# Juzhan/TAP-Net

Hardware: AMD Instinct MI355X
Metric: env-steps/s (batch placements) 2D n=10 LB_GREEDY; 1/2/4/8 GPU + CPU ref (higher is better)
Workload: dtype i32 height-maps / f64 candidate scores / f32 masks

## Files before the change

tap-net_amd/csrc/tap_masks.h:

```cpp
#pragma once

#include <hip/hip_runtime.h>

#include <cstdint>
#include <type_traits>
#include <cstdlib>

#include "tap_stream_variant.h"

constexpr size_t TAP_WT_MAX_BYTES = 64u << 20;

struct MaskArgs {
    int B, n, R, nR, rows, update_rows, static_rows;
    const float *dyn_in;
    float *dyn_out;
    const float *static_;
    const int64_t *ptr;
    const float *mask_in;
    const float *cs_in;
    float *cs_out;
    float *cur_out;
    float *mask_out;
    const unsigned long long *bits_in;
    unsigned long long *bits_out;
// ... 176 lines not shown
{
    const int nR = a.nR;
    const size_t slab = (size_t)a.rows * nR;
    const int nchunk = (int)(slab / 4);
    int total = 0;
#pragma unroll
    for (int k = 0; k < NS; ++k) if (on[k]) total = (k + 1) * nchunk;
    if (total == 0) return;
    long p[NS];
    float row0[NS][NC], cs[NS][NC][3], keep[NS][NC];
#pragma unroll
    for (int k = 0; k < NS; ++k) {
        const int env = senv0 + k;
        p[k] = on[k] ? (long)a.ptr[env] : 0;
#pragma unroll
        for (int c = 0; c < NC; ++c) {
            const int j = lane + 64 * c;
            const bool ok = on[k] && j < nR;
            row0[k][c] = ok ? a.static_[(size_t)env * a.static_rows * nR + j] : 0.f;
            keep[k][c] = ok ? (a.mask_in ? a.mask_in[(size_t)env * nR + j] : 1.f) : 0.f;
#pragma unroll
            for (int s = 0; s < 3; ++s) cs[k][c][s] = ok ? a.cs_in[((size_t)env * 3 + s) * nR + j] : 0.f;
        }
    }
    for (int i = lane; i < NS * 3 * nR; i += 64) lds[i] = 0.f;

    const float4 *s4 = reinterpret_cast<const float4 *>(a.dyn_in + (size_t)senv0 * slab);
    float4 *d4 = reinterpret_cast<float4 *>(a.dyn_out + (size_t)senv0 * slab);
    ClearRanges cr[NS];
    bool have_real = false;
    for (int base = 0; base < total; base += 64 * U) {
        float4 v[U];
#pragma unroll
        for (int u = 0; u < U; ++u) v[u] = s4[min(base + u * 64 + lane, total - 1)];
        if (!have_real) {
#pragma unroll
            for (int k = 0; k < NS; ++k) {
                float r0 = -1.f;
#pragma unroll
                for (int c = 0; c < NC; ++c) {
                    const float t = __shfl(row0[k][c], (int)(p[k] & 63));
                    if ((p[k] >> 6) == c && p[k] >= 0 && p[k] < nR) r0 = t;
                }
                cr[k] = clear_ranges(a, on[k] ? (long)r0 : -1);
            }
            have_real = true;
        }
#pragma unroll
        for (int u = 0; u < U; ++u) {
            const int q = base + u * 64 + lane;
            if (q < total) {
                const int k = (NS > 1 && q >= nchunk) ? 1 : 0;
                const int f = (q - k * nchunk) * 4;
#pragma unroll
                for (int s = 0; s < 3; ++s)
                    if (f >= cr[k].lo[s] && f < cr[k].hi[s]) {
                        *reinterpret_cast<float4 *>(lds + (k * 3 + s) * nR + (f - cr[k].lo[s])) = v[u];
                        v[u] = make_float4(0.f, 0.f, 0.f, 0.f);
                    }
                d4[q] = v[u];
            }
        }
    }
    __builtin_amdgcn_fence(__ATOMIC_RELEASE, "wavefront");
    __builtin_amdgcn_wave_barrier();
    __builtin_amdgcn_fence(__ATOMIC_ACQUIRE, "wavefront");
#pragma unroll
    for (int k = 0; k < NS; ++k) {
        if (!on[k]) continue;
        const int env = senv0 + k;
        const long real_m = (p[k] >= 0 && p[k] < nR) ? tap_mod_col(p[k], a.n, a.nR) : -1 - (long)a.n * a.R;
#pragma unroll
        for (int c = 0; c < NC; ++c) {
            const int j = lane + 64 * c;
            if (j >= nR) continue;
            float sum[3];
#pragma unroll
            for (int s = 0; s < 3; ++s) {
                sum[s] = cs[k][c][s] - lds[(k * 3 + s) * nR + j];
                if (a.cs_out) a.cs_out[((size_t)env * 3 + s) * nR + j] = sum[s];
            }
            float kp = keep[k][c];
            for (int r = 0; r < a.R; ++r)
                if (j == real_m + (long)a.n * r) kp = 0.f;
            if (a.mask_out) a.mask_out[(size_t)env * nR + j] = kp;
            const float dm = sum[1] * sum[2] + sum[0];
            if (a.cur_out) a.cur_out[(size_t)env * nR + j] = dm != 0.f ? 0.f : kp;
        }
    }
}

template <int NS>
__device__ __forceinline__ void stream_build_bits(const MaskArgs &a, int senv0, int lane, const bool (&on)[NS],
                                                  unsigned long long *tile )
{
    typedef unsigned long long u64;
    const int nR = a.nR, C4 = nR >> 2, rows = a.rows;
    const int rsub = (int)(((unsigned)lane * (unsigned)a.c4_magic) >> 16), c4 = lane - rsub * C4, RP = a.rp;
    for (int i = lane; i < NS * nR; i += 64) tile[i] = 0ull;
    tap_wave_lds_sync_m();
    int bad = 0;
    constexpr int U = 4;
    for (int r0 = rsub; r0 < rows; r0 += U * RP) {
        float4 v[NS][U];
#pragma unroll
        for (int k = 0; k < NS; ++k) {
            const float4 *src = reinterpret_cast<const float4 *>(a.dyn_in + (size_t)(senv0 + (on[k] ? k : 0)) * rows * nR) + c4;
#pragma unroll
            for (int u = 0; u < U; ++u) v[k][u] = src[(size_t)min(r0 + u * RP, rows - 1) * C4];
        }
#pragma unroll
        for (int k = 0; k < NS; ++k) {
            unsigned lo[4] = {0u, 0u, 0u, 0u}, hi[4] = {0u, 0u, 0u, 0u};
#pragma unroll
            for (int u = 0; u < U; ++u) {
                const int r = r0 + u * RP;
                if (r >= rows || rsub >= RP || !on[k]) continue;
                const float e[4] = {v[k][u].x, v[k][u].y, v[k][u].z, v[k][u].w};
#pragma unroll
                for (int q = 0; q < 4; ++q) {
                    const unsigned nz = e[q] != 0.f;
                    bad += (nz && e[q] != 1.f);
                    if (r < 32) lo[q] |= nz << r; else hi[q] |= nz << (r - 32);
                }
            }
            if (on[k] && rsub < RP) {
#pragma unroll
                for (int q = 0; q < 4; ++q) {
                    const u64 word = ((u64)hi[q] << 32) | lo[q];
                    if (word) atomicOr(&tile[k * nR + c4 * 4 + q], word);
                }
            }
        }
    }
    if (a.nonbinary) {
        const unsigned long long any = __ballot(bad != 0);
        if (any) {
#pragma unroll
            for (int o = 32; o > 0; o >>= 1) bad += __shfl_xor(bad, o);
            if (lane == 0) atomicAdd(a.nonbinary, bad);
        }
    }
    tap_wave_lds_sync_m();
}

__device__ __forceinline__ int tap_mod_small(int v, int n)
{
#pragma unroll
    for (int r = 0; r < 5; ++r) v = v >= n ? v - n : v;
    while (v >= n) v -= n;
    return v;
}

template <int NS, int NC, bool BUILD = false, bool MERGED = true, int C4S = 0, bool INPLACE = false, bool FULL = false>
__device__ __forceinline__ void stream_wave_bits_r4(const MaskArgs &a, int senv0, int lane, const bool (&on_)[NS],
                                                 float *lds = nullptr)
{
    static_assert(!(BUILD && INPLACE), "the first step on a fresh tensor writes all of it");
    bool on[NS];
#pragma unroll
    for (int k = 0; k < NS; ++k) on[k] = FULL ? true : on_[k];
#if defined(TAP_STREAM_LOAD_BJ)
    constexpr bool BJ_X = false;
#elif defined(TAP_STREAM_BJX_ALL)
    constexpr bool BJ_X = !BUILD && NC == 1 && (C4S == 5 || C4S == 15);
#else
    constexpr bool BJ_X = !BUILD && NC == 1 && NS == 1 && (C4S == 5 || C4S == 15);
#endif
    typedef unsigned long long u64;
    static_assert(NS <= 2, "a stream wave expands one or two slabs");
    if (!on[0]) return;
    const int nR = C4S ? 4 * C4S : a.nR, C4 = C4S ? C4S : nR >> 2, rows = C4S ? (C4S == 10 ? 60 : 30) : a.rows, n = C4S ? (C4S == 10 ? 20 : 10) : a.n;
    const int RP = C4S ? 64 / C4S : a.rp;
    const int c4_magic = C4S ? 65536 / C4S + 1 : a.c4_magic;
    const bool lane_on = lane < RP * C4;
#ifdef TAP_STREAM_UNALIGNED
    const LaneRole role = stream_lane_role(lane, 0, C4, RP, c4_magic, 0, 0, 0);
#else
    const LaneRole role = stream_lane_role(lane, senv0, C4, RP, c4_magic, a.sb_mul, a.sb_add, 0);
#endif
    const bool first_row = role.rsub == 0;
    u64 *tile = reinterpret_cast<u64 *>(lds);
    const void *any = BUILD ? static_cast<const void *>(a.dyn_in) : static_cast<const void *>(a.bits_in);
    const bool has_ptr = FULL || a.ptr != nullptr, has_static = FULL || a.static_ != nullptr, has_mask = FULL || a.mask_in != nullptr;
    const int64_t *ptrp = has_ptr ? a.ptr : static_cast<const int64_t *>(any);
    const float *stp = has_static ? a.static_ : static_cast<const float *>(any);
    const float *mip = has_mask ? a.mask_in : static_cast<const float *>(any);
    long praw[NS];
    float row0[NS][NC], keep[NS][NC];
    u64 bj[NS][NC];
    ulonglong2 w[NS][2];
#pragma unroll
    for (int k = 0; k < NS; ++k) {
        const int env = on[k] ? senv0 + k : senv0;
        praw[k] = ptrp[has_ptr ? env : 0];
        const float *strow = stp + (has_static ? (size_t)env * a.static_rows * nR : (size_t)0);
        const float *mirow = mip + (has_mask ? (size_t)env * nR : (size_t)0);
#pragma unroll
        for (int c = 0; c < NC; ++c) {
            const unsigned j = (unsigned)min(lane + 64 * c, nR - 1);
            row0[k][c] = strow[has_static ? j : 0u];
            keep[k][c] = mirow[has_mask ? j : 0u];
        }
    }
#ifdef TAP_STREAM_G2
    __builtin_amdgcn_s_waitcnt(0x0F70);
#endif
    if (!BUILD) {
#pragma unroll
        for (int k = 0; k < NS; ++k) {
            const int env = on[k] ? senv0 + k : senv0;
            const unsigned long long *brow = a.bits_in + (size_t)env * nR;
            if constexpr (!BJ_X) {
#pragma unroll
                for (int c = 0; c < NC; ++c) bj[k][c] = brow[(unsigned)min(lane + 64 * c, nR - 1)];
            }
            const ulonglong2 *src = reinterpret_cast<const ulonglong2 *>(brow) + (unsigned)(role.c4 * 2);
            w[k][0] = src[0];
            w[k][1] = src[1];
        }
    }
    if (BUILD) {
        stream_build_bits<NS>(a, senv0, lane, on, tile);
#pragma unroll
        for (int k = 0; k < NS; ++k) {
#pragma unroll
            for (int c = 0; c < NC; ++c) bj[k][c] = tile[(size_t)k * nR + min(lane + 64 * c, nR - 1)];
            const ulonglong2 *src = reinterpret_cast<const ulonglong2 *>(tile + (size_t)k * nR + role.c4 * 4);
            w[k][0] = src[0];
            w[k][1] = src[1];
        }
    }
    float *o_dyn = a.dyn_out, *o_cur = a.cur_out, *o_mask = a.mask_out;
    unsigned long long *o_bits = a.bits_out;
    int o_wt = a.wt;
#ifdef TAP_STREAM_EARLY_ARGS
    asm volatile("" : "+s"(o_dyn), "+s"(o_cur), "+s"(o_mask), "+s"(o_bits), "+s"(o_wt));
#endif
    __builtin_amdgcn_s_waitcnt(0x0F70);
#ifdef TAP_PROF
    TL_STAMP(1);
#endif
    const u64 nmask = (n >= 64) ? ~0ull : ((1ull << n) - 1ull);
    auto mod_n = [&](int v) -> int {
        if constexpr (C4S != 0) return (int)((unsigned)v % (unsigned)(C4S == 10 ? 20 : 10));
        else return tap_mod_small(v, n);
    };
    int jm[NC];
#pragma unroll
    for (int c = 0; c < NC; ++c) jm[c] = mod_n(min(lane + 64 * c, nR - 1));
    u64 clr[NS];
    int pm[NS], realk[NS];
    constexpr int UR_C = C4S != 0 ? 3 : 0;
    const int ur = UR_C ? UR_C : a.update_rows;
#pragma unroll
    for (int k = 0; k < NS; ++k) {
        const bool valid_v = on[k] && has_ptr && praw[k] >= 0 && praw[k] < nR;
#ifdef TAP_STREAM_VPICK
        constexpr bool SPICK = false;
#else
        constexpr bool SPICK = NS > 1;
#endif
        bool valid;
        int p, real;
        if constexpr (!SPICK) {
            valid = valid_v;
            p = valid ? (int)praw[k] : 0;
            float r0 = -1.f;
#pragma unroll
            for (int c = 0; c < NC; ++c) {
                const float t = __shfl(row0[k][c], p & 63);
                if (valid && has_static && (p >> 6) == c) r0 = t;
            }
            real = (r0 > -1.f && r0 < (float)rows) ? (int)r0 : -1;
        } else {
            const int ps = __builtin_amdgcn_readfirstlane(valid_v ? (int)praw[k] : -1);
            valid = ps >= 0;
            p = valid ? ps : 0;
            float r0 = -1.f;
#pragma unroll
            for (int c = 0; c < NC; ++c) {
                const float t = __int_as_float(__builtin_amdgcn_readlane(__float_as_int(row0[k][c]), p & 63));
                if (valid && has_static && (p >> 6) == c) r0 = t;
            }
            real = __builtin_amdgcn_readfirstlane((r0 > -1.f && r0 < (float)rows) ? (int)r0 : -1);
        }
        u64 m = 0;
#pragma unroll
        for (int i = 0; i < 3; ++i) {
            const int r = real + n * i;
            if (i < ur && real >= 0 && r < rows) m |= 1ull << r;
        }
        clr[k] = m;
        realk[k] = real;
        pm[k] = valid ? mod_n(p) : -1;
    }
    u64 nw[NS][4];
#pragma unroll
    for (int k = 0; k < NS; ++k) {
        nw[k][0] = w[k][0].x & ~clr[k]; nw[k][1] = w[k][0].y & ~clr[k];
        nw[k][2] = w[k][1].x & ~clr[k]; nw[k][3] = w[k][1].y & ~clr[k];
    }
    if constexpr (INPLACE) {
        if (o_dyn) {
            const float4 z = make_float4(0.f, 0.f, 0.f, 0.f);
            const int total = ur * C4;
            for (int idx = lane; idx < total; idx += 64) {
                const int i = (idx * c4_magic) >> 16, c = idx - i * C4;
#pragma unroll
                for (int k = 0; k < NS; ++k) {
                    const int r = realk[k] + n * i;
                    if (!on[k] || realk[k] < 0 || r >= rows) continue;
                    float4 *dst = reinterpret_cast<float4 *>(o_dyn) + ((size_t)(senv0 + k) * rows + r) * C4 + c;
#if defined(TAP_INPLACE_STORE) && TAP_INPLACE_STORE == 1
                    store_stream(dst, z, o_wt);
#elif defined(TAP_INPLACE_STORE) && TAP_INPLACE_STORE == 2
                    *dst = z;
#else
                    if (o_wt) store_stream(dst, z, 1); else *dst = z;
#endif
                }
            }
        }
    }
    if (lane_on) {
        if (!INPLACE && o_dyn) {
            const int non = (NS > 1 && on[NS - 1]) ? 2 : 1;
            const int total = non * rows;
            const int nq = (C4S ? (non * rows + RP - 1) / RP : (non > 1 ? a.nq2 : a.nq)) + role.nq;
            float4 *dst = reinterpret_cast<float4 *>(o_dyn + (size_t)senv0 * rows * nR) + role.c4;
            int rr = role.r0;
            bool done = false;
            if constexpr (NS > 1 && !MERGED) {
                if (rows <= 32) {
#pragma unroll
                    for (int k = 0; k < NS; ++k) {
                        if (!on[k]) continue;
                        float4 *dk = dst + (size_t)k * rows * C4;
                        const unsigned m0 = (unsigned)nw[k][0], m1 = (unsigned)nw[k][1], m2 = (unsigned)nw[k][2], m3 = (unsigned)nw[k][3];
                        for (int r = role.rsub; r < rows; r += RP) {
                            const float4 v = make_float4((float)((m0 >> r) & 1u), (float)((m1 >> r) & 1u),
                                                         (float)((m2 >> r) & 1u), (float)((m3 >> r) & 1u));
                            store_stream(&dk[(size_t)r * C4], v, o_wt);
                        }
                    }
                    done = true;
                }
            }
            if (done) {
            } else if (C4S != 0 && rows <= 32) {
                constexpr int ROWS_C = 30, RP_C = C4S ? 64 / C4S : 1, NQC = (NS * ROWS_C + RP_C - 1) / RP_C + 1;
                auto run = [&](auto wt_c) {
#pragma unroll
                    for (int i = 0; i < NQC; ++i) {
                        const int ri = rr + RP_C * i;
                        if ((unsigned)ri >= (unsigned)total) continue;
                        const bool up = NS > 1 && ri >= ROWS_C;
                        const int r = up ? ri - ROWS_C : ri;
                        const unsigned m0 = up ? (unsigned)nw[NS - 1][0] : (unsigned)nw[0][0], m1 = up ? (unsigned)nw[NS - 1][1] : (unsigned)nw[0][1],
                                       m2 = up ? (unsigned)nw[NS - 1][2] : (unsigned)nw[0][2], m3 = up ? (unsigned)nw[NS - 1][3] : (unsigned)nw[0][3];
                        const float4 v = make_float4((float)((m0 >> r) & 1u), (float)((m1 >> r) & 1u),
                                                     (float)((m2 >> r) & 1u), (float)((m3 >> r) & 1u));
                        store_stream(&dst[(size_t)ri * C4], v, decltype(wt_c)::value);
                    }
                };
#ifdef TAP_STREAM_ROLLED
                for (int i = 0; i < nq; ++i, rr += RP) {
                    if ((unsigned)rr >= (unsigned)total) continue;
                    const bool up = NS > 1 && rr >= rows;
                    const int r = up ? rr - rows : rr;
                    const unsigned m0 = up ? (unsigned)nw[NS - 1][0] : (unsigned)nw[0][0], m1 = up ? (unsigned)nw[NS - 1][1] : (unsigned)nw[0][1],
                                   m2 = up ? (unsigned)nw[NS - 1][2] : (unsigned)nw[0][2], m3 = up ? (unsigned)nw[NS - 1][3] : (unsigned)nw[0][3];
                    const float4 v = make_float4((float)((m0 >> r) & 1u), (float)((m1 >> r) & 1u),
                                                 (float)((m2 >> r) & 1u), (float)((m3 >> r) & 1u));
                    store_stream(&dst[(size_t)rr * C4], v, o_wt);
                }
#else
                if (o_wt) run(std::integral_constant<int, 1>{}); else run(std::integral_constant<int, 0>{});
#endif
            } else if (rows <= 32) {
                for (int i = 0; i < nq; ++i, rr += RP) {
                    if ((unsigned)rr >= (unsigned)total) continue;
                    const bool up = NS > 1 && rr >= rows;
                    const int r = up ? rr - rows : rr;
                    const unsigned m0 = up ? (unsigned)nw[NS - 1][0] : (unsigned)nw[0][0], m1 = up ? (unsigned)nw[NS - 1][1] : (unsigned)nw[0][1],
                                   m2 = up ? (unsigned)nw[NS - 1][2] : (unsigned)nw[0][2], m3 = up ? (unsigned)nw[NS - 1][3] : (unsigned)nw[0][3];
                    const float4 v = make_float4((float)((m0 >> r) & 1u), (float)((m1 >> r) & 1u),
                                                 (float)((m2 >> r) & 1u), (float)((m3 >> r) & 1u));
                    store_stream(&dst[(size_t)rr * C4], v, o_wt);
                }
            } else {
                for (int i = 0; i < nq; ++i, rr += RP) {
                    if ((unsigned)rr >= (unsigned)total) continue;
                    const bool up = NS > 1 && rr >= rows;
                    const int r = up ? rr - rows : rr;
                    const float4 v = make_float4(bit_as_float(up ? nw[NS - 1][0] : nw[0][0], r), bit_as_float(up ? nw[NS - 1][1] : nw[0][1], r),
                                                 bit_as_float(up ? nw[NS - 1][2] : nw[0][2], r), bit_as_float(up ? nw[NS - 1][3] : nw[0][3], r));
                    store_stream(&dst[(size_t)rr * C4], v, o_wt);
                }
            }
        }
        if (first_row && o_bits) {
#pragma unroll
            for (int k = 0; k < NS; ++k) {
                if (!on[k]) continue;
                ulonglong2 *dst = reinterpret_cast<ulonglong2 *>(o_bits + (size_t)(senv0 + k) * nR + role.c4 * 4);
                dst[0] = make_ulonglong2(nw[k][0], nw[k][1]);
                dst[1] = make_ulonglong2(nw[k][2], nw[k][3]);
            }
        }
    }
    unsigned nbx[NS];
    if constexpr (BJ_X) {
        const int jj = min(lane, nR - 1);
        const int src = ((jj >> 2) + role.sb) << 2;
        const int e = jj & 3;
#pragma unroll
        for (int k = 0; k < NS; ++k) {
            const int e0 = __builtin_amdgcn_ds_bpermute(src, (int)(unsigned)nw[k][0]), e1 = __builtin_amdgcn_ds_bpermute(src, (int)(unsigned)nw[k][1]);
            const int e2 = __builtin_amdgcn_ds_bpermute(src, (int)(unsigned)nw[k][2]), e3 = __builtin_amdgcn_ds_bpermute(src, (int)(unsigned)nw[k][3]);
            nbx[k] = (unsigned)(e == 0 ? e0 : e == 1 ? e1 : e == 2 ? e2 : e3);
        }
    }
#pragma unroll
    for (int k = 0; k < NS; ++k) {
        if (!on[k]) continue;
        const int env = senv0 + k;
#pragma unroll
        for (int c = 0; c < NC; ++c) {
            const int j = lane + 64 * c;
            if (j >= nR) continue;
            const u64 nb = BJ_X ? (u64)nbx[k] : (bj[k][c] & ~clr[k]);
            const int move = __popcll(nb & nmask), small = n >= 64 ? 0 : __popcll((nb >> n) & nmask);
            const int large = n >= 32 ? 0 : __popcll((nb >> (2 * n)) & nmask);
            const float kp = (jm[c] == pm[k]) ? 0.f : (has_mask ? keep[k][c] : 1.f);
            if (o_mask) o_mask[(size_t)env * nR + j] = kp;
            if (o_cur) o_cur[(size_t)env * nR + j] = (small * large + move) != 0 ? 0.f : kp;
        }
    }
}

#ifdef TAP_STREAM_R3
template <int NS, int NC, bool BUILD = false>
__device__ __forceinline__ void stream_wave_bits_r3(const MaskArgs &a, int senv0, int lane, const bool (&on)[NS],
                                                 float *lds = nullptr)
{
    typedef unsigned long long u64;
    const int nR = a.nR, C4 = nR >> 2, rows = a.rows;
    const int rsub = (int)(((unsigned)lane * (unsigned)a.c4_magic) >> 16), c4 = lane - rsub * C4, RP = a.rp;
    const bool lane_on = rsub < RP;
    constexpr bool build = BUILD;
    u64 *tile = reinterpret_cast<u64 *>(lds);
    long p[NS];
    float row0[NS][NC], keep[NS][NC];
    u64 bj[NS][NC];
    ulonglong2 w[NS][2];
#pragma unroll
    for (int k = 0; k < NS; ++k) {
        const int env = senv0 + k;
        p[k] = (on[k] && a.ptr) ? (long)a.ptr[env] : -1;
#pragma unroll
        for (int c = 0; c < NC; ++c) {
            const int j = lane + 64 * c;
            const bool ok = on[k] && j < nR;
            row0[k][c] = (ok && a.static_) ? a.static_[(size_t)env * a.static_rows * nR + j] : 0.f;
            keep[k][c] = ok ? (a.mask_in ? a.mask_in[(size_t)env * nR + j] : 1.f) : 0.f;
        }
    }
    if (BUILD) stream_build_bits<NS>(a, senv0, lane, on, tile);
#pragma unroll
    for (int k = 0; k < NS; ++k) {
        const int env = senv0 + k;
        const size_t wbase = build ? (size_t)k * nR : (size_t)env * nR;
#pragma unroll
        for (int c = 0; c < NC; ++c) {
            const int j = lane + 64 * c;
            const bool ok = on[k] && j < nR;
            if (BUILD) bj[k][c] = ok ? tile[wbase + j] : 0ull;
            else bj[k][c] = ok ? a.bits_in[wbase + j] : 0ull;
        }
        const bool ok = on[k] && lane_on;
        if (BUILD) {
            const ulonglong2 *src = reinterpret_cast<const ulonglong2 *>(tile + wbase + c4 * 4);
            w[k][0] = ok ? src[0] : make_ulonglong2(0, 0);
            w[k][1] = ok ? src[1] : make_ulonglong2(0, 0);
        } else {
            const ulonglong2 *src = reinterpret_cast<const ulonglong2 *>(a.bits_in + wbase + c4 * 4);
            w[k][0] = ok ? src[0] : make_ulonglong2(0, 0);
            w[k][1] = ok ? src[1] : make_ulonglong2(0, 0);
        }
    }
    const u64 nmask = (a.n >= 64) ? ~0ull : ((1ull << a.n) - 1ull);
#pragma unroll
    for (int k = 0; k < NS; ++k) {
        if (!on[k]) continue;
        const int env = senv0 + k;
        float r0 = -1.f;
#pragma unroll
        for (int c = 0; c < NC; ++c) {
            const float t = __shfl(row0[k][c], (int)(p[k] & 63));
            if ((p[k] >> 6) == c && p[k] >= 0 && p[k] < nR) r0 = t;
        }
        const long real = (long)r0;
        u64 clr = 0;
        for (int i = 0; i < a.update_rows; ++i) {
            const long r = real + (long)a.n * i;
            if (real >= 0 && r < rows) clr |= 1ull << r;
        }
        if (lane_on) {
            const u64 n0 = w[k][0].x & ~clr, n1 = w[k][0].y & ~clr, n2 = w[k][1].x & ~clr, n3 = w[k][1].y & ~clr;
#ifdef TAP_PROF
            if (k == 0) { TL_WAIT_VM(); TL_STAMP(1); }
#endif
            if (a.dyn_out) {
                float4 *dst = reinterpret_cast<float4 *>(a.dyn_out + (size_t)env * rows * nR) + c4;
                if (rows <= 32) {
                    const unsigned m0 = (unsigned)n0, m1 = (unsigned)n1, m2 = (unsigned)n2, m3 = (unsigned)n3;
                    for (int r = rsub; r < rows; r += RP) {
                        const float4 v = make_float4((float)((m0 >> r) & 1u), (float)((m1 >> r) & 1u),
                                                     (float)((m2 >> r) & 1u), (float)((m3 >> r) & 1u));
                        store_stream(&dst[(size_t)r * C4], v, a.wt);
                    }
                } else {
                    for (int r = rsub; r < rows; r += RP) {
                        const float4 v = make_float4(bit_as_float(n0, r), bit_as_float(n1, r), bit_as_float(n2, r),
                                                     bit_as_float(n3, r));
                        store_stream(&dst[(size_t)r * C4], v, a.wt);
                    }
                }
            }
            if (rsub == 0 && a.bits_out) {
                ulonglong2 *dst = reinterpret_cast<ulonglong2 *>(a.bits_out + (size_t)env * nR + c4 * 4);
                dst[0] = make_ulonglong2(n0, n1);
                dst[1] = make_ulonglong2(n2, n3);
            }
        }
        const long real_m = (p[k] >= 0 && p[k] < nR) ? tap_mod_col(p[k], a.n, a.nR) : -1 - (long)a.n * a.R;
#pragma unroll
        for (int c = 0; c < NC; ++c) {
            const int j = lane + 64 * c;
            if (j >= nR) continue;
            const u64 nb = bj[k][c] & ~clr;
            const int move = __popcll(nb & nmask), small = a.n >= 64 ? 0 : __popcll((nb >> a.n) & nmask);
            const int large = a.n >= 32 ? 0 : __popcll((nb >> (2 * a.n)) & nmask);
            float kp = keep[k][c];
            for (int r = 0; r < a.R; ++r)
                if (j == real_m + (long)a.n * r) kp = 0.f;
            if (a.mask_out) a.mask_out[(size_t)env * nR + j] = kp;
            if (a.cur_out) a.cur_out[(size_t)env * nR + j] = (small * large + move) != 0 ? 0.f : kp;
        }
    }
}

#endif
template <int NS, int NC, bool BUILD = false, bool MERGED = true, int C4S = 0, bool INPLACE = false, bool FULL = false>
__device__ __forceinline__ void stream_wave_bits(const MaskArgs &a, int senv0, int lane, const bool (&on)[NS], float *lds = nullptr)
{
#ifdef TAP_STREAM_R3
    stream_wave_bits_r3<NS, NC, BUILD>(a, senv0, lane, on, lds);
#else
    stream_wave_bits_r4<NS, NC, BUILD, MERGED, C4S, INPLACE, FULL>(a, senv0, lane, on, lds);
#endif
}

__host__ __device__ __forceinline__ int mask_bit_planes(int rows) { return rows > 64 ? 2 : 1; }

__device__ __forceinline__ unsigned long long bits_range64(int a, int b)
{
    a = a < 0 ? 0 : a;
    b = b > 64 ? 64 : b;
    if (a >= b) return 0ull;
    return ((b - a) >= 64 ? ~0ull : ((1ull << (b - a)) - 1ull)) << a;
}

template <int NC, bool BUILD>
__device__ __forceinline__ void stream_wave_bits2(const MaskArgs &a, int env, int lane, float *lds)
{
    typedef unsigned long long u64;
    const int nR = a.nR, C4 = nR >> 2, rows = a.rows;
    const int rsub = (int)(((unsigned)lane * (unsigned)a.c4_magic) >> 16), c4 = lane - rsub * C4, RP = a.rp;
    const bool lane_on = rsub < RP;
    u64 *tile = reinterpret_cast<u64 *>(lds);
    const long p = a.ptr ? (long)a.ptr[env] : -1;
    float row0[NC], keep[NC];
#pragma unroll
    for (int c = 0; c < NC; ++c) {
        const int j = lane + 64 * c;
        const bool ok = j < nR;
        row0[c] = (ok && a.static_) ? a.static_[(size_t)env * a.static_rows * nR + j] : 0.f;
        keep[c] = ok ? (a.mask_in ? a.mask_in[(size_t)env * nR + j] : 1.f) : 0.f;
    }
    if (BUILD) {
        for (int i = lane; i < 2 * nR; i += 64) tile[i] = 0ull;
        tap_wave_lds_sync_m();
        int bad = 0;
        constexpr int U = 4;
        const float4 *src = reinterpret_cast<const float4 *>(a.dyn_in + (size_t)env * rows * nR) + c4;
        u64 acc[2][4] = {{0ull, 0ull, 0ull, 0ull}, {0ull, 0ull, 0ull, 0ull}};
        for (int r0 = rsub; r0 < rows; r0 += U * RP) {
            float4 v[U];
#pragma unroll
            for (int u = 0; u < U; ++u) v[u] = src[(size_t)min(r0 + u * RP, rows - 1) * C4];
#pragma unroll
            for (int u = 0; u < U; ++u) {
                const int r = r0 + u * RP;
                if (r >= rows || !lane_on) continue;
                const float e[4] = {v[u].x, v[u].y, v[u].z, v[u].w};
#pragma unroll
                for (int q = 0; q < 4; ++q) {
                    const u64 nz = e[q] != 0.f;
                    bad += (nz && e[q] != 1.f);
                    if (r < 64) acc[0][q] |= nz << r; else acc[1][q] |= nz << (r - 64);
                }
            }
        }
        if (lane_on) {
#pragma unroll
            for (int w = 0; w < 2; ++w)
#pragma unroll
                for (int q = 0; q < 4; ++q)
                    if (acc[w][q]) atomicOr(&tile[w * nR + c4 * 4 + q], acc[w][q]);
        }
        if (a.nonbinary) {
            const unsigned long long any = __ballot(bad != 0);
            if (any) {
#pragma unroll
                for (int o = 32; o > 0; o >>= 1) bad += __shfl_xor(bad, o);
                if (lane == 0) atomicAdd(a.nonbinary, bad);
            }
        }
        tap_wave_lds_sync_m();
    }
    const u64 *win = BUILD ? tile : a.bits_in + (size_t)env * 2 * nR;
    const LaneRole role = stream_lane_role(lane, env, C4, RP, a.c4_magic, a.sb_mul, a.sb_add, a.nq);
    u64 bj[NC][2], w4[2][4];
#pragma unroll
    for (int c = 0; c < NC; ++c) {
        const int j = lane + 64 * c;
#pragma unroll
        for (int w = 0; w < 2; ++w) bj[c][w] = j < nR ? win[w * nR + j] : 0ull;
    }
#pragma unroll
    for (int w = 0; w < 2; ++w) {
        const ulonglong2 *src = reinterpret_cast<const ulonglong2 *>(win + w * nR + role.c4 * 4);
        const ulonglong2 s0 = lane_on ? src[0] : make_ulonglong2(0, 0), s1 = lane_on ? src[1] : make_ulonglong2(0, 0);
        w4[w][0] = s0.x; w4[w][1] = s0.y; w4[w][2] = s1.x; w4[w][3] = s1.y;
    }
    float r0 = -1.f;
#pragma unroll
    for (int c = 0; c < NC; ++c) {
        const float t = __shfl(row0[c], (int)(p & 63));
        if ((p >> 6) == c && p >= 0 && p < nR) r0 = t;
    }
    const long real = (long)r0;
    u64 clr[2] = {0ull, 0ull};
    for (int i = 0; i < a.update_rows; ++i) {
        const long r = real + (long)a.n * i;
        if (real >= 0 && r < rows) { if (r < 64) clr[0] |= 1ull << r; else clr[1] |= 1ull << (r - 64); }
    }
    if (lane_on) {
#pragma unroll
        for (int w = 0; w < 2; ++w)
#pragma unroll
            for (int q = 0; q < 4; ++q) w4[w][q] &= ~clr[w];
        if (a.dyn_out) {
            float4 *dst = reinterpret_cast<float4 *>(a.dyn_out + (size_t)env * rows * nR) + role.c4;
            int r = role.r0;
            for (int i = 0; i < role.nq; ++i, r += RP) {
                if ((unsigned)r >= (unsigned)rows) continue;
                const bool up = r >= 64;
                const int rb = r & 63;
                const float4 v = make_float4(bit_as_float(up ? w4[1][0] : w4[0][0], rb), bit_as_float(up ? w4[1][1] : w4[0][1], rb),
                                             bit_as_float(up ? w4[1][2] : w4[0][2], rb), bit_as_float(up ? w4[1][3] : w4[0][3], rb));
                store_stream(&dst[(size_t)r * C4], v, a.wt);
            }
        }
        if (role.rsub == 0 && a.bits_out) {
#pragma unroll
            for (int w = 0; w < 2; ++w) {
                ulonglong2 *dst = reinterpret_cast<ulonglong2 *>(a.bits_out + ((size_t)env * 2 + w) * nR + role.c4 * 4);
                dst[0] = make_ulonglong2(w4[w][0], w4[w][1]);
                dst[1] = make_ulonglong2(w4[w][2], w4[w][3]);
            }
        }
    }
    const long real_m = (p >= 0 && p < nR) ? tap_mod_col(p, a.n, a.nR) : -1 - (long)a.n * a.R;
    const int n = a.n;
#pragma unroll
    for (int c = 0; c < NC; ++c) {
        const int j = lane + 64 * c;
        if (j >= nR) continue;
        const u64 lo = bj[c][0] & ~clr[0], hi = bj[c][1] & ~clr[1];
        int sec[3];
#pragma unroll
        for (int s = 0; s < 3; ++s)
            sec[s] = __popcll(lo & bits_range64(s * n, (s + 1) * n)) + __popcll(hi & bits_range64(s * n - 64, (s + 1) * n - 64));
        float kp = keep[c];
        for (int r = 0; r < a.R; ++r)
            if (j == real_m + (long)n * r) kp = 0.f;
        if (a.mask_out) a.mask_out[(size_t)env * nR + j] = kp;
        if (a.cur_out) a.cur_out[(size_t)env * nR + j] = (sec[1] * sec[2] + sec[0]) != 0 ? 0.f : kp;
    }
}

inline bool mask_bits_ok(const MaskArgs &a)
{
    return (a.bits_in || mask_builds_bits(a)) && (a.ptr == nullptr || a.static_ != nullptr) && (a.nR % 4 == 0) &&
           a.nR <= 256 && a.rows >= 1 && a.rows <= 128 &&
           ((reinterpret_cast<uintptr_t>(a.dyn_out) | reinterpret_cast<uintptr_t>(a.dyn_in)) % 16 == 0) &&
           ((reinterpret_cast<uintptr_t>(a.bits_in) | reinterpret_cast<uintptr_t>(a.bits_out)) % 16 == 0);
}

inline int mask_fast_path_cols(const MaskArgs &a)
{
    if (a.bits_in || mask_builds_bits(a)) return a.nR <= 64 ? 1 : a.nR <= 128 ? 2 : 4;
// ... 11 lines not shown
```

tap-net_amd/csrc/tap_transition.h:

```cpp
#pragma once

#include "tap_common.h"
#include "tap_masks.h"
#include "tap_place.h"

constexpr int TAP_T_PROF_NOSTREAM = 1 << 8, TAP_T_PROF_NOPLACE = 1 << 9;

struct TransArgs {
    StepArgs s;
    MaskArgs m;
    int flags;
    float *ratio_out;
};

template <int SPW, int NC, int MODE_>
__device__ __forceinline__ void trans_stream_wave(const MaskArgs &m, int senv0, int lane, float *lds)
{
    constexpr int MODE = MODE_ & 3;
    constexpr bool MERGED = (MODE_ & TAP_MODE_MERGED) != 0;
    constexpr bool INPLACE = (MODE_ & TAP_MODE_INPLACE) != 0, FULL = (MODE_ & TAP_MODE_FULL) != 0;
    static_assert(!INPLACE || MODE == 1, "in place: only on a shadow the caller hands in");
    constexpr int C4S = (MODE_ & TAP_MODE_C4_10) == TAP_MODE_C4_10 ? 10 : (MODE_ & TAP_MODE_C4_5) ? 5 : (MODE_ & TAP_MODE_C4_15) ? 15 : 0;
    static_assert(C4S == 0 || NC == 1, "the compiled-in window shapes have one column per lane");
    bool on[SPW];
#pragma unroll
    for (int k = 0; k < SPW; ++k) on[k] = senv0 + k < m.B;
    TL_STAMP(0);
    if (NC > 0) {
        if (MODE == 1) stream_wave_bits<SPW, (NC > 0 ? NC : 1), false, MERGED, C4S, INPLACE, FULL>(m, senv0, lane, on, lds);
        else if (MODE == 2) stream_wave_bits<SPW, (NC > 0 ? NC : 1), true, MERGED, C4S>(m, senv0, lane, on, lds);
        else stream_wave_fast<SPW, (NC > 2 ? 4 : 6), (NC > 0 ? NC : 1)>(m, senv0, lane, on, lds);
        TL_STAMP(2);
        TL_WAIT_VM();
        TL_STAMP(3);
        return;
    }
    const size_t slab = (size_t)m.rows * m.nR;
#pragma unroll
    for (int k = 0; k < SPW; ++k) {
        if (!on[k]) continue;
        const int senv = senv0 + k;
        bool badp;
        const long pc = tap_col((long)m.ptr[senv], m.nR, badp);
        const long real = badp ? -1 : (long)m.static_[(size_t)senv * m.static_rows * m.nR + pc];
        const long p = badp ? -1 : pc;
        const ClearRanges cr = clear_ranges(m, real);
        const float *src = m.dyn_in + (size_t)senv * slab;
        float *dst = m.dyn_out + (size_t)senv * slab;
        for (long f = lane; f < (long)slab; f += 64) {
            float v = src[f];
            if (in_cleared(cr, (int)f)) v = 0.f;
            dst[f] = v;
        }
        mask_env(m, senv, lane, real, p);
    }
}

template <int G, int SW> struct TransGeom {
    static constexpr int EPB = (G == 64) ? 4 : 8;
    static constexpr int ENV_WAVES = EPB * G / 64;
    static constexpr int STREAM_WAVES = (SW < EPB) ? SW : EPB;
    static constexpr int SPW = EPB / STREAM_WAVES;
    static constexpr int THREADS = 64 * (ENV_WAVES + STREAM_WAVES);
};
```

tap-net_amd/csrc/transition.hip:

```cpp
#include <cstdlib>
#include <new>

#include "tap_common.h"
#include "tap_macs.h"
#include "tap_macs3.h"
#include "tap_masks.h"
#include "tap_place.h"
#include "tap_transition.h"
#include "tap_waves.h"

template <int D, int G, int NC, int SW, int MODE>
__global__ void __launch_bounds__((TransGeom<G, SW>::THREADS)) k_transition(TAP_MASK_HOT_PARAMS, TransArgs a)
{
    using Geo = TransGeom<G, SW>;
    constexpr int EPB = Geo::EPB, SPW = Geo::SPW, ENV_WAVES = Geo::ENV_WAVES;
    extern __shared__ float trans_lds[];
    __shared__ int s_old[64 * ENV_WAVES];
    __shared__ int s_new[64 * ENV_WAVES];
    const int tid = threadIdx.x, lane = tid & 63;
#ifdef TAP_VWAVE
    const int wave = tid >> 6;
#else
    const int wave = TransGeom<G, SW>::SPW > 1 ? __builtin_amdgcn_readfirstlane(tid >> 6) : tid >> 6;
#endif
    const int env_base = blockIdx.x * EPB;

#if defined(TAP_PROF) || defined(TAP_PROF_SWITCH)
    if (wave >= ENV_WAVES ? (a.flags & TAP_T_PROF_NOSTREAM) : (a.flags & TAP_T_PROF_NOPLACE)) return;
#endif
    if (wave >= ENV_WAVES) {
#ifdef TAP_STREAM_PRIO
        __builtin_amdgcn_s_setprio(TAP_STREAM_PRIO);
#endif
        const MaskArgs m = tap_mask_hot(a.m, (MODE & 3) == 1, TAP_MASK_HOT_NAMES);
        trans_stream_wave<SPW, NC, MODE>(m, env_base + (wave - ENV_WAVES) * SPW, lane,
                                     trans_lds + (size_t)(wave - ENV_WAVES) * SPW * 3 * h_nR);
        return;
    }

#ifdef TAP_PLACE_PRIO
    __builtin_amdgcn_s_setprio(TAP_PLACE_PRIO);
#else
    __builtin_amdgcn_s_setprio(2);
#endif
    const int cell = tid % G;
    TL_STAMP(0);
    StepArgs sa = a.s;
    sa.ptr = h_ptr; sa.static_ = h_static; sa.nR = h_nR; sa.static_rows = h_static_rows; sa.d.B = h_B;
    tap_lb_place_wave<D, G>(sa, a.flags, a.ratio_out, env_base + tid / G, cell, lane,
                            s_old + (tid - cell), s_new + (tid - cell));
    TL_WAIT_VM();
    TL_STAMP(3);
}

#ifdef TAP_PROF
extern "C" int tap_prof_read_timeline(unsigned long long *out, int clear)
{
    (void)hipMemcpyFromSymbol(out, HIP_SYMBOL(tap_prof_tl), sizeof(unsigned long long) * TAP_PROF_WGS * TAP_PROF_WAVES * 4);
    if (clear) {
        static unsigned long long zeros[TAP_PROF_WGS * TAP_PROF_WAVES * 4];
        (void)hipMemcpyToSymbol(HIP_SYMBOL(tap_prof_tl), zeros, sizeof(zeros));
    }
    return 0;
}
#endif

int tap_transition_macs_launch(tap_ctx *ctx, const tap_env_desc *d, const TransArgs &a, hipStream_t st);
bool tap_big_transition_ok(const tap_ctx *ctx, const tap_env_desc *d, int nR);
int tap_big_transition(tap_ctx *ctx, const tap_env_desc *d, const TransArgs &a, hipStream_t st);
bool tap_macs_wave_transition_ok(const tap_ctx *ctx, const tap_env_desc *d, int nR);
int tap_macs_wave_transition(tap_ctx *ctx, const tap_env_desc *d, const TransArgs &a, hipStream_t st);
bool tap_macs3_wave_transition_ok(const tap_ctx *ctx, const tap_env_desc *d, int nR);
int tap_macs3_wave_transition(tap_ctx *ctx, const tap_env_desc *d, const TransArgs &a, hipStream_t st);
int tap_macs2d_wave_from();

static int transition_wave_kind(const tap_ctx *ctx, const tap_env_desc *d, int nR, int rows)
{
    if (rows > 64) return 0;
    if (tap_is_big(d)) return tap_big_transition_ok(ctx, d, nR) ? 1 : 0;
    if (d->strategy != TAP_MACS) return 0;
    if (d->D == 2) return (d->W > 16 && d->W >= tap_macs2d_wave_from() && tap_macs_wave_transition_ok(ctx, d, nR)) ? 2 : 0;
    return (tap_is_big_macs3(d) && tap_macs3_wave_transition_ok(ctx, d, nR)) ? 3 : 0;
}

static int transition_wave_launch(tap_ctx *ctx, const tap_env_desc *d, void *state, const TransArgs &a, int kind, void *stream)
{
    if (kind == 1) return tap_big_transition(ctx, d, a, (hipStream_t)stream);
    int rc = TAP_OK;
    if ((a.flags & TAP_T_FRESH) && (rc = tap_env_reset(ctx, d, state, stream)) != TAP_OK) return rc;
    rc = kind == 2 ? tap_macs_wave_transition(ctx, d, a, (hipStream_t)stream) : tap_macs3_wave_transition(ctx, d, a, (hipStream_t)stream);
    if (rc == TAP_OK && (a.flags & TAP_T_RATIO)) rc = tap_env_ratio(ctx, d, state, a.ratio_out, nullptr, nullptr, stream);
    return rc;
}
int tap_macs_validate(tap_ctx *ctx, const tap_env_desc &d);

template <int D, int G, int SW>
static int launch_transition_v(tap_ctx *ctx, const TransArgs &a, hipStream_t st)
{
    constexpr int EPB = TransGeom<G, SW>::EPB, THREADS = TransGeom<G, SW>::THREADS;
    const int grid = (a.s.d.B + EPB - 1) / EPB;
    if (grid == 0) return TAP_OK;
    const size_t lds = (size_t)EPB * 3 * a.m.nR * sizeof(float);
    const TapVariant v = tap_stream_variant(TAP_SV_TRANSITION, tap_mask_facts(a.m), TapLaunchFacts{D, G, EPB, a.s.d.B, 0, 0, false});
    return tap_launch_variant<TAP_SV_TRANSITION, D, G>(ctx, "k_transition", v, a.m.wt, [&](auto k) -> int {
        using K = decltype(k);
        hipLaunchKernelGGL((k_transition<D, G, K::nc, SW, K::mode>), dim3(grid), dim3(THREADS), K::nc ? lds : 0, st,
                           TAP_MASK_HOT_ARGS(a.m), a);
        return TAP_OK;
    });
}

template <int D, int G> static int launch_transition(tap_ctx *ctx, const TransArgs &a, hipStream_t st)
{
#ifdef TAP_TRANS_SW
    return launch_transition_v<D, G, TAP_TRANS_SW>(ctx, a, st);
#else
    return launch_transition_v<D, G, (D == 3 ? 8 : 4)>(ctx, a, st);
#endif
}

static int transition_dispatch(tap_ctx *ctx, const tap_env_desc *d, const TransArgs &a, void *stream);

static bool transition_single_kernel(const tap_ctx *ctx, const tap_env_desc *d, int nR)
{
    if (d->strategy == TAP_LB || tap_is_big(d) || tap_is_big_macs3(d) || (d->strategy == TAP_MACS && d->D == 2 && d->W > 16)) return false;
    if (d->strategy == TAP_MACS) {
        const int G = tap_group_size(d), epb = G == 64 ? 4 : 8;
        const size_t words = d->D == 3 ? (size_t)macs3_group_words(G, d->n_max, d->H)
                                       : (size_t)macs_group_words(d->W <= 8 ? 8 : 16, d->H, d->n_max, d->W);
        if ((size_t)epb * 3 * nR * sizeof(float) + (size_t)epb * words * sizeof(int) > tap_lds_limit(ctx)) return false;
    }
    return true;
}

struct StepAux {
    float *dec_static_out;
    int64_t *tour_out;
    int tour_stride, tour_col;
};

__global__ void __launch_bounds__(TAP_BLOCK) k_step_aux(StepArgs s)
{
    const int env = blockIdx.x * TAP_BLOCK + threadIdx.x;
    if (env >= s.d.B) return;
    bool badp;
    const long praw = (long)s.ptr[env];
    const long p = tap_col(praw, s.nR, badp);
    float fv[3] = {0.f, 0.f, 0.f};
    for (int k = 0; k < s.d.D; ++k) {
        const float v = s.static_[((size_t)env * s.static_rows + 1 + k) * s.nR + p];
        fv[k] = badp ? 0.f : v;
    }
    tap_step_aux(s, env, s.d.D, fv, praw);
}

int tap_step_aux_launch(tap_ctx *ctx, const StepArgs &s, hipStream_t st)
{
    if (!(s.dec_static_out || s.tour_out || s.picked_out) || s.d.B == 0) return TAP_OK;
    hipLaunchKernelGGL(k_step_aux, dim3((s.d.B + TAP_BLOCK - 1) / TAP_BLOCK), dim3(TAP_BLOCK), 0, st, s);
    TAP_LAUNCH_CHECK(ctx, "k_step_aux");
    return TAP_OK;
}

extern "C" int tap_transition_launches(const tap_ctx *ctx, const tap_env_desc *d, int n, int R, int rows, int on_bits)
{
    if (!d || n < 1 || R < 1 || rows < 1) return TAP_E_INVALID;
    if (on_bits && transition_wave_kind(ctx, d, n * R, rows)) return 1;
    return (transition_single_kernel(ctx, d, n * R) && (!on_bits || rows <= 64)) ? 1 : 2;
}

static int transition_tail(tap_ctx *ctx, const tap_env_desc *d, void *state, const TransArgs &a, void *stream)
{
    int rc = tap_env_step_gather(ctx, d, state, a.s.static_, a.s.static_rows, a.s.nR, a.s.ptr, nullptr, a.s.feature_out, stream);
    if (rc == TAP_OK && (a.flags & TAP_T_RATIO)) rc = tap_env_ratio(ctx, d, state, a.ratio_out, nullptr, nullptr, stream);
    return rc ? rc : tap_step_aux_launch(ctx, a.s, (hipStream_t)stream);
}

static int transition_common(tap_ctx *ctx, const tap_env_desc *d, void *state, int n, int R, int rows,
                             int update_rows, const float *static_, int static_rows, const int64_t *ptr,
                             const float *mask_in, float *current_out, float *mask_out, float *feature_out,
                             float *ratio_out, int flags, TransArgs &a, const StepAux *aux = nullptr)
{
    int rc = tap_desc_validate(ctx, d);
    if (rc) return rc;
    if (d->B == 0) return TAP_OK;
    if (d->strategy == TAP_MACS && (rc = tap_macs_validate(ctx, *d)) != TAP_OK) return rc;
    if (!state || !static_ || !ptr || (!mask_in && !aux) || !current_out || !mask_out || n < 1 || R < 1 || rows < 1 ||
        static_rows < 1 + d->D || update_rows < 0 || update_rows > 3 || ((flags & TAP_T_RATIO) && !ratio_out))
        return tap_fail(ctx, TAP_E_INVALID, "bad transition arguments");
    a.s.d = *d;
    tap_env_layout(d, state, &a.s.v);
    a.s.static_ = static_; a.s.static_rows = static_rows; a.s.nR = n * R; a.s.ptr = ptr;
    a.s.feature_out = feature_out; a.s.flen = tap_env_feature_len(d);
    a.s.lut = ctx ? ctx->stab_lut : nullptr;
    a.flags = flags;
    a.ratio_out = ratio_out;
    if (aux) {
        a.s.dec_static_out = aux->dec_static_out;
        a.s.tour_out = aux->tour_out;
        a.s.tour_stride = aux->tour_stride;
        a.s.tour_col = aux->tour_col;
    }
    return TAP_OK;
}

static int transition_copy_impl(tap_ctx *ctx, const tap_env_desc *d, void *state, int n, int R, int rows,
                                int update_rows, const float *dyn_in, const float *static_,
                                int static_rows, const int64_t *ptr, const float *mask_in,
                                const float *colsum_in, float *dyn_out, float *colsum_out,
                                float *current_out, float *mask_out, float *feature_out,
                                float *ratio_out, int flags, void *stream, const StepAux *aux)
{
    if (d && d->B == 0) return tap_desc_validate(ctx, d);
    TransArgs a = {};
    int rc = transition_common(ctx, d, state, n, R, rows, update_rows, static_, static_rows, ptr, mask_in,
                               current_out, mask_out, feature_out, ratio_out, flags, a, aux);
    if (rc) return rc;
    if (!dyn_in || !colsum_in || !dyn_out || !colsum_out)
        return tap_fail(ctx, TAP_E_INVALID, "bad transition arguments");
    if (dyn_in == dyn_out) return tap_fail(ctx, TAP_E_INVALID, "transition is out of place (pack.py:370)");
    if (!transition_single_kernel(ctx, d, n * R)) {
        if ((flags & TAP_T_FRESH) && (rc = tap_env_reset(ctx, d, state, stream)) != TAP_OK) return rc;
        rc = tap_mask_step(ctx, d->B, n, R, rows, update_rows, dyn_in, static_, static_rows, ptr, mask_in, colsum_in, dyn_out,
                           colsum_out, current_out, mask_out, stream);
        return rc ? rc : transition_tail(ctx, d, state, a, stream);
    }
    a.m = mask_finish(MaskArgs{d->B, n, R, n * R, rows, update_rows, static_rows, dyn_in, dyn_out, static_, ptr,
                   mask_in, colsum_in, colsum_out, current_out, mask_out, nullptr, nullptr});
    return transition_dispatch(ctx, d, a, stream);
}

extern "C" int tap_transition(tap_ctx *ctx, const tap_env_desc *d, void *state, int n, int R, int rows,
                              int update_rows, const float *dyn_in, const float *static_,
                              int static_rows, const int64_t *ptr, const float *mask_in,
                              const float *colsum_in, float *dyn_out, float *colsum_out,
                              float *current_out, float *mask_out, float *feature_out,
                              float *ratio_out, int flags, void *stream)
{
    if (d && d->B > 0 && !mask_in) return tap_fail(ctx, TAP_E_INVALID, "bad transition arguments");
    return transition_copy_impl(ctx, d, state, n, R, rows, update_rows, dyn_in, static_, static_rows, ptr, mask_in, colsum_in,
                                dyn_out, colsum_out, current_out, mask_out, feature_out, ratio_out, flags, stream, nullptr);
}

static int transition_bits_impl(tap_ctx *ctx, const tap_env_desc *d, void *state, int n, int R, int rows,
                                int update_rows, const unsigned long long *bits_in, const float *static_,
                                int static_rows, const int64_t *ptr, const float *mask_in,
                                unsigned long long *bits_out, float *dyn_out, float *current_out,
                                float *mask_out, float *feature_out, float *ratio_out, int flags,
                                void *stream, const StepAux *aux, int inplace = 0)
{
    if (d && d->B == 0) return tap_desc_validate(ctx, d);
    TransArgs a = {};
    int rc = transition_common(ctx, d, state, n, R, rows, update_rows, static_, static_rows, ptr, mask_in,
                               current_out, mask_out, feature_out, ratio_out, flags, a, aux);
    if (rc) return rc;
    if (!bits_in || !bits_out || bits_in == bits_out)
        return tap_fail(ctx, TAP_E_INVALID, "bad transition_bits arguments");
    if (const int kind = transition_wave_kind(ctx, d, n * R, rows)) {
        a.m = mask_finish(MaskArgs{d->B, n, R, n * R, rows, update_rows, static_rows, nullptr, dyn_out, static_, ptr,
// ... 236 lines not shown
```

Measured before the change: 1.479 billion.

## Split mask/cur-mask output into a dedicated extra wave in 2D transition kernel

For the 2D n=10 FULL merged stream variant, adds a separate 64-lane wave per block that computes update_mask and current-mask outputs with vectorized float4 loads and stores, one lane per env/column quad. The stream waves are compiled with NOMASK so they skip the mask loads and the mask tail. The aim is to shorten the critical stream-wave path by running the mask work in parallel. In exchange each block gets one more wave, which can affect occupancy, and some inputs (ptr, static row, bits) are read twice.

```diff
diff --git a/tap-net_amd/csrc/tap_masks.h b/tap-net_amd/csrc/tap_masks.h
--- a/tap-net_amd/csrc/tap_masks.h
+++ b/tap-net_amd/csrc/tap_masks.h
@@ -352,11 +352,12 @@
     return v;
 }
 
-template <int NS, int NC, bool BUILD = false, bool MERGED = true, int C4S = 0, bool INPLACE = false, bool FULL = false>
+template <int NS, int NC, bool BUILD = false, bool MERGED = true, int C4S = 0, bool INPLACE = false, bool FULL = false, bool NOMASK = false>
 __device__ __forceinline__ void stream_wave_bits_r4(const MaskArgs &a, int senv0, int lane, const bool (&on_)[NS],
                                                  float *lds = nullptr)
 {
     static_assert(!(BUILD && INPLACE), "the first step on a fresh tensor writes all of it");
+    static_assert(!NOMASK || (FULL && !BUILD && C4S != 0), "the mask wave exists beside the FULL step on a compiled-in shape only");
     bool on[NS];
 #pragma unroll
     for (int k = 0; k < NS; ++k) on[k] = FULL ? true : on_[k];
@@ -400,7 +401,7 @@
         for (int c = 0; c < NC; ++c) {
             const unsigned j = (unsigned)min(lane + 64 * c, nR - 1);
             row0[k][c] = strow[has_static ? j : 0u];
-            keep[k][c] = mirow[has_mask ? j : 0u];
+            if constexpr (!NOMASK) keep[k][c] = mirow[has_mask ? j : 0u];
         }
     }
 #ifdef TAP_STREAM_G2
@@ -411,7 +412,7 @@
         for (int k = 0; k < NS; ++k) {
             const int env = on[k] ? senv0 + k : senv0;
             const unsigned long long *brow = a.bits_in + (size_t)env * nR;
-            if constexpr (!BJ_X) {
+            if constexpr (!BJ_X && !NOMASK) {
 #pragma unroll
                 for (int c = 0; c < NC; ++c) bj[k][c] = brow[(unsigned)min(lane + 64 * c, nR - 1)];
             }
@@ -610,6 +611,7 @@
             }
         }
     }
+    if constexpr (NOMASK) return;
     unsigned nbx[NS];
     if constexpr (BJ_X) {
         const int jj = min(lane, nR - 1);
@@ -753,14 +755,63 @@
 }
 
 #endif
-template <int NS, int NC, bool BUILD = false, bool MERGED = true, int C4S = 0, bool INPLACE = false, bool FULL = false>
+template <int NS, int NC, bool BUILD = false, bool MERGED = true, int C4S = 0, bool INPLACE = false, bool FULL = false, bool NOMASK = false>
 __device__ __forceinline__ void stream_wave_bits(const MaskArgs &a, int senv0, int lane, const bool (&on)[NS], float *lds = nullptr)
 {
 #ifdef TAP_STREAM_R3
+    static_assert(!NOMASK, "the round-3 stream wave always carries update_mask");
     stream_wave_bits_r3<NS, NC, BUILD>(a, senv0, lane, on, lds);
 #else
-    stream_wave_bits_r4<NS, NC, BUILD, MERGED, C4S, INPLACE, FULL>(a, senv0, lane, on, lds);
-#endif
+    stream_wave_bits_r4<NS, NC, BUILD, MERGED, C4S, INPLACE, FULL, NOMASK>(a, senv0, lane, on, lds);
+#endif
+}
+
+typedef float tap_f4u __attribute__((ext_vector_type(4), aligned(4)));
+template <int EPB, int C4S>
+__device__ __forceinline__ void mask_wave_bits(const MaskArgs &a, int env0, int lane)
+{
+    static_assert(C4S == 5 && EPB * C4S <= 64, "one lane per (env, column quad) of the 10-node 2D window");
+    constexpr int nR = 4 * C4S, n = 10, rows = 30;
+    TL_STAMP(0);
+    if (lane >= EPB * C4S) return;
+    const int e = lane / C4S, q = lane - e * C4S;
+    const int env = env0 + e;
+    const long praw = (long)a.ptr[env];
+    const tap_f4u keep = *reinterpret_cast<const tap_f4u *>(a.mask_in + (size_t)env0 * nR + lane * 4);
+    const ulonglong2 *wsrc = reinterpret_cast<const ulonglong2 *>(a.bits_in + (size_t)env0 * nR) + lane * 2;
+    const ulonglong2 w0 = wsrc[0], w1 = wsrc[1];
+    const bool valid = praw >= 0 && praw < nR;
+    const int p = valid ? (int)praw : 0;
+    const float r0v = a.static_[(size_t)env * a.static_rows * nR + p];
+    const float r0 = valid ? r0v : -1.f;
+    const int real = (r0 > -1.f && r0 < (float)rows) ? (int)r0 : -1;
+    unsigned clr = 0;
+#pragma unroll
+    for (int i = 0; i < 3; ++i) {
+        const int r = real + n * i;
+        if (real >= 0 && r < rows) clr |= 1u << r;
+    }
+    const int pm = valid ? (int)((unsigned)p % (unsigned)n) : -1;
+    const unsigned nmask = (1u << n) - 1u;
+    const unsigned word[4] = {(unsigned)w0.x, (unsigned)w0.y, (unsigned)w1.x, (unsigned)w1.y};
+    tap_f4u kp, cur;
+#pragma unroll
+    for (int c = 0; c < 4; ++c) {
+        const int j = q * 4 + c, jm = j >= n ? j - n : j;
+        const unsigned nb = word[c] & ~clr;
+        const int move = __popc(nb & nmask), small = __popc((nb >> n) & nmask), large = __popc((nb >> (2 * n)) & nmask);
+        kp[c] = (jm == pm) ? 0.f : keep[c];
+        cur[c] = (small * large + move) != 0 ? 0.f : kp[c];
+    }
+#ifdef TAP_PROF
+    TL_WAIT_VM();
+    TL_STAMP(1);
+#endif
+    *reinterpret_cast<tap_f4u *>(a.mask_out + (size_t)env0 * nR + lane * 4) = kp;
+    *reinterpret_cast<tap_f4u *>(a.cur_out + (size_t)env0 * nR + lane * 4) = cur;
+    TL_STAMP(2);
+    TL_WAIT_VM();
+    TL_STAMP(3);
 }
 
 __host__ __device__ __forceinline__ int mask_bit_planes(int rows) { return rows > 64 ? 2 : 1; }
diff --git a/tap-net_amd/csrc/tap_transition.h b/tap-net_amd/csrc/tap_transition.h
--- a/tap-net_amd/csrc/tap_transition.h
+++ b/tap-net_amd/csrc/tap_transition.h
@@ -13,7 +13,7 @@
     float *ratio_out;
 };
 
-template <int SPW, int NC, int MODE_>
+template <int SPW, int NC, int MODE_, bool NOMASK = false>
 __device__ __forceinline__ void trans_stream_wave(const MaskArgs &m, int senv0, int lane, float *lds)
 {
     constexpr int MODE = MODE_ & 3;
@@ -27,7 +27,7 @@
     for (int k = 0; k < SPW; ++k) on[k] = senv0 + k < m.B;
     TL_STAMP(0);
     if (NC > 0) {
-        if (MODE == 1) stream_wave_bits<SPW, (NC > 0 ? NC : 1), false, MERGED, C4S, INPLACE, FULL>(m, senv0, lane, on, lds);
+        if (MODE == 1) stream_wave_bits<SPW, (NC > 0 ? NC : 1), false, MERGED, C4S, INPLACE, FULL, NOMASK>(m, senv0, lane, on, lds);
         else if (MODE == 2) stream_wave_bits<SPW, (NC > 0 ? NC : 1), true, MERGED, C4S>(m, senv0, lane, on, lds);
         else stream_wave_fast<SPW, (NC > 2 ? 4 : 6), (NC > 0 ? NC : 1)>(m, senv0, lane, on, lds);
         TL_STAMP(2);
@@ -63,3 +63,16 @@
     static constexpr int SPW = EPB / STREAM_WAVES;
     static constexpr int THREADS = 64 * (ENV_WAVES + STREAM_WAVES);
 };
+
+template <int D, int G, int NC, int SW, int MODE> constexpr bool trans_mask_wave()
+{
+#ifdef TAP_NO_MASK_WAVE
+    return false;
+#else
+    return D == 2 && NC == 1 && TransGeom<G, SW>::SPW == 2 && MODE == (1 | TAP_MODE_MERGED | TAP_MODE_C4_5 | TAP_MODE_FULL);
+#endif
+}
+template <int D, int G, int NC, int SW, int MODE> constexpr int trans_threads()
+{
+    return TransGeom<G, SW>::THREADS + (trans_mask_wave<D, G, NC, SW, MODE>() ? 64 : 0);
+}
diff --git a/tap-net_amd/csrc/transition.hip b/tap-net_amd/csrc/transition.hip
--- a/tap-net_amd/csrc/transition.hip
+++ b/tap-net_amd/csrc/transition.hip
@@ -10,10 +10,11 @@
 #include "tap_waves.h"
 
 template <int D, int G, int NC, int SW, int MODE>
-__global__ void __launch_bounds__((TransGeom<G, SW>::THREADS)) k_transition(TAP_MASK_HOT_PARAMS, TransArgs a)
+__global__ void __launch_bounds__((trans_threads<D, G, NC, SW, MODE>())) k_transition(TAP_MASK_HOT_PARAMS, TransArgs a)
 {
     using Geo = TransGeom<G, SW>;
     constexpr int EPB = Geo::EPB, SPW = Geo::SPW, ENV_WAVES = Geo::ENV_WAVES;
+    constexpr bool MASKW = trans_mask_wave<D, G, NC, SW, MODE>();
     extern __shared__ float trans_lds[];
     __shared__ int s_old[64 * ENV_WAVES];
     __shared__ int s_new[64 * ENV_WAVES];
@@ -33,8 +34,14 @@
         __builtin_amdgcn_s_setprio(TAP_STREAM_PRIO);
 #endif
         const MaskArgs m = tap_mask_hot(a.m, (MODE & 3) == 1, TAP_MASK_HOT_NAMES);
-        trans_stream_wave<SPW, NC, MODE>(m, env_base + (wave - ENV_WAVES) * SPW, lane,
-                                     trans_lds + (size_t)(wave - ENV_WAVES) * SPW * 3 * h_nR);
+        if constexpr (MASKW) {
+            if (wave == ENV_WAVES + Geo::STREAM_WAVES) {
+                mask_wave_bits<EPB, 5>(m, env_base, lane);
+                return;
+            }
+        }
+        trans_stream_wave<SPW, NC, MODE, MASKW>(m, env_base + (wave - ENV_WAVES) * SPW, lane,
+                                            trans_lds + (size_t)(wave - ENV_WAVES) * SPW * 3 * h_nR);
         return;
     }
 
@@ -97,14 +104,14 @@
 template <int D, int G, int SW>
 static int launch_transition_v(tap_ctx *ctx, const TransArgs &a, hipStream_t st)
 {
-    constexpr int EPB = TransGeom<G, SW>::EPB, THREADS = TransGeom<G, SW>::THREADS;
+    constexpr int EPB = TransGeom<G, SW>::EPB;
     const int grid = (a.s.d.B + EPB - 1) / EPB;
     if (grid == 0) return TAP_OK;
     const size_t lds = (size_t)EPB * 3 * a.m.nR * sizeof(float);
     const TapVariant v = tap_stream_variant(TAP_SV_TRANSITION, tap_mask_facts(a.m), TapLaunchFacts{D, G, EPB, a.s.d.B, 0, 0, false});
     return tap_launch_variant<TAP_SV_TRANSITION, D, G>(ctx, "k_transition", v, a.m.wt, [&](auto k) -> int {
         using K = decltype(k);
-        hipLaunchKernelGGL((k_transition<D, G, K::nc, SW, K::mode>), dim3(grid), dim3(THREADS), K::nc ? lds : 0, st,
+        hipLaunchKernelGGL((k_transition<D, G, K::nc, SW, K::mode>), dim3(grid), dim3(trans_threads<D, G, K::nc, SW, K::mode>()), K::nc ? lds : 0, st,
                            TAP_MASK_HOT_ARGS(a.m), a);
         return TAP_OK;
     });
```

After: 1.523 billion (median of 6 runs). 3.0% higher.
